# espnet/espnet

Measured on AMD Instinct MI355X. Metric: audio-seconds/sec (RTF^-1), Conformer-ASR, 10 s utterances, higher is better.
Workload: dtype bf16; 1 GPU; BASELINE.json configs[1]: Conformer-small (12x256d, 4 heads), HIP STFT/log-mel + HIP encoder + greedy CTC (G1) + hypotheses collated to the host, 32 x 10 s utterances per GPU per step, V=5000; batch_per_gpu=32, global_batch=32, parallelism=utterance-dp1

## Files before the change

### espnet_amd/csrc/api.hip

```cpp
#include <stdlib.h>

#include <atomic>
#include <mutex>

#include "em_common.h"
#include "switches.h"

namespace {
EmSwitches read_switches() {
  auto on = [](const char* n) { return getenv(n) != nullptr; };
  auto num = [](const char* n, int dflt) { const char* e = getenv(n); return e ? atoi(e) : dflt; };
  EmSwitches s = {};
  s.attn2_stamps = on("EM_ATTN2_STAMPS"); s.block_stamps = on("EM_BLOCK_STAMPS"); s.ffn_stamps = on("EM_FFN_STAMPS");
  s.sub2_stamps = on("EM_SUB2_STAMPS");
  s.block_no_helpers = on("ESPNET_AMD_BLOCK_NO_HELPERS");
  s.sa_split = num("ESPNET_AMD_SA_SPLIT", 0); s.sa_group = num("ESPNET_AMD_SA_GROUP", 0);
  s.no_sa_tree = on("ESPNET_AMD_NO_SA_TREE"); s.sa_tree_min_rows = num("ESPNET_AMD_SA_TREE_MIN_ROWS", 200);
  s.no_attn2_large = on("ESPNET_AMD_NO_ATTN2_LARGE"); s.no_ffn_rows = on("ESPNET_AMD_NO_FFN_ROWS");
  s.no_rows_ctc = on("ESPNET_AMD_NO_ROWS_CTC"); s.frontend_v1 = on("ESPNET_AMD_FRONTEND_V1");
  s.gemm_stages = num("ESPNET_AMD_GEMM_STAGES", 0); s.gemm_bm = num("ESPNET_AMD_GEMM_BM", 0); s.no_mid_gemm = on("ESPNET_AMD_NO_MID_GEMM");
  s.mid_tile = num("ESPNET_AMD_MID_TILE", 0); s.lng_rt = num("ESPNET_AMD_LNG_RT", 0); s.lng_wide = num("ESPNET_AMD_LNG_WIDE", 256);
  s.no_src_lnq = on("ESPNET_AMD_NO_SRC_LNQ"); s.no_tail_fusion = on("ESPNET_AMD_NO_TAIL_FUSION");
  s.stream_no_fused = on("ESPNET_AMD_STREAM_NO_FUSED"); s.stream_mha_v1 = on("ESPNET_AMD_STREAM_MHA_V1");
  s.stream_no_ctx_fold = on("ESPNET_AMD_STREAM_NO_CTX_FOLD"); s.stream_no_ln_gemm = on("ESPNET_AMD_STREAM_NO_LN_GEMM");
  s.stream_fused_min = num("ESPNET_AMD_STREAM_FUSED_MIN", 1); s.no_sub12 = on("ESPNET_AMD_NO_SUB12");
  s.stream_ffn_split = num("ESPNET_AMD_STREAM_FFN_SPLIT", 0); s.stream_split_att = on("ESPNET_AMD_STREAM_SPLIT_ATT");
  s.stream_tf_merge = num("ESPNET_AMD_STREAM_TF_MERGE", -1);
  s.dec_ffn_split = num("ESPNET_AMD_DEC_FFN_SPLIT", 0); s.dec_ffn_rows = num("ESPNET_AMD_DEC_FFN_ROWS", 0); s.no_rows_qkv = on("ESPNET_AMD_NO_ROWS_QKV"); s.ffn_rows_min_fill = num("ESPNET_AMD_FFN_ROWS_MIN_FILL", 0);
  return s;
}
std::atomic<const EmSwitches*> g_sw{nullptr};
std::mutex g_sw_mu;
}

const EmSwitches& em_sw() {
  const EmSwitches* p = g_sw.load(std::memory_order_acquire);
  if (!p) {
    std::lock_guard<std::mutex> lk(g_sw_mu);
    p = g_sw.load(std::memory_order_acquire);
    if (!p) {
      p = new EmSwitches(read_switches());
      g_sw.store(p, std::memory_order_release);
    }
  }
  return *p;
}
extern "C" void em_dev_switches_reload(void) {
  std::lock_guard<std::mutex> lk(g_sw_mu);
  g_sw.store(new EmSwitches(read_switches()), std::memory_order_release);
}

extern "C" int em_version(void) { return 1; }

extern "C" const char* em_error_string(int code) {
  switch (code) {
    case EM_OK: return "ok";
    case EM_ERR_UNSUPPORTED: return "shape/config outside the MI355X fast path";
    case EM_ERR_BAD_ARG: return "bad argument";
    case EM_ERR_TOO_SHORT: return "utterance too short for Conv2dSubsampling (needs >= 7 frames)";
    case EM_ERR_LAUNCH: return "HIP kernel launch failed";
    case EM_ERR_WORKSPACE: return "workspace too small";
    case EM_ERR_IO: return "file I/O failed";
  }
  return "unknown error";
}

template <typename T>
__global__ void cast_f32_kernel(const float* __restrict__ src, size_t n, T* __restrict__ dst) {
  size_t i = (size_t)blockIdx.x * blockDim.x + threadIdx.x;
  const size_t stride = (size_t)gridDim.x * blockDim.x;
  for (; i < n; i += stride) dst[i] = from_f32<T>(src[i]);
}

extern "C" int em_cast_f32(int dtype, const float* src, size_t n, void* dst, void* stream) {
  if (!src || !dst) return EM_ERR_BAD_ARG;
  if (n == 0) return EM_OK;
  int blocks = (int)((n + 255) / 256);
  if (blocks > 4096) blocks = 4096;
  if (dtype == EM_F32)
    hipLaunchKernelGGL(cast_f32_kernel<float>, dim3(blocks), dim3(256), 0, (hipStream_t)stream, src,
                       n, (float*)dst);
  else if (dtype == EM_BF16)
    hipLaunchKernelGGL(cast_f32_kernel<bf16>, dim3(blocks), dim3(256), 0, (hipStream_t)stream, src,
                       n, (bf16*)dst);
  else
    return EM_ERR_BAD_ARG;
  EM_CHECK_LAUNCH();
  return EM_OK;
}
```

### espnet_amd/csrc/frontend.hip

```cpp
#include <stdlib.h>

#include "em_common.h"
#include <type_traits>
#include "switches.h"

__device__ const float2 EM_TW512[384] = {
#include "twiddle512.inc"
};

__device__ __forceinline__ float2 cmul(float2 a, float2 b) {
  return make_float2(a.x * b.x - a.y * b.y, a.x * b.y + a.y * b.x);
}

__device__ __forceinline__ void bfly4(float2 u[4]) {
  float2 a = make_float2(u[0].x + u[2].x, u[0].y + u[2].y);
  float2 b = make_float2(u[0].x - u[2].x, u[0].y - u[2].y);
  float2 c = make_float2(u[1].x + u[3].x, u[1].y + u[3].y);
  float2 d = make_float2(u[1].x - u[3].x, u[1].y - u[3].y);
  u[0] = make_float2(a.x + c.x, a.y + c.y);
  u[2] = make_float2(a.x - c.x, a.y - c.y);
  u[1] = make_float2(b.x + d.y, b.y - d.x);
  u[3] = make_float2(b.x - d.y, b.y + d.x);
}

__device__ __forceinline__ int reflect_idx(int p, int N) {
  if (p < 0) p = -p;
  if (p >= N) p = 2 * (N - 1) - p;
  return p;
}

__global__ __launch_bounds__(256) void frontend_logmel_kernel(
    const float* __restrict__ wav, int N, int hop, const float* __restrict__ window,
    const float* __restrict__ melw, const int* __restrict__ mel_lo, int mel_maxlen, int n_mels,
    const int* __restrict__ flens, const int* __restrict__ wlens, int T_f,
    float* __restrict__ feats) {
  __shared__ float s_re[4][2][256];
  __shared__ float s_im[4][2][256];
  __shared__ float s_pow[4][264];
  const int wave = threadIdx.x >> 6, lane = threadIdx.x & 63;
  const int b = blockIdx.y;
  const int t_raw = blockIdx.x * 4 + wave;
  const int t = t_raw < T_f ? t_raw : T_f - 1;
  const float* x = wav + (size_t)b * N;
  const int Nb = wlens ? (wlens[b] < N ? wlens[b] : N) : N;
  float(*re)[256] = s_re[wave];
  float(*im)[256] = s_im[wave];

  float2 u[4];
  const int start = t * hop - 256;
#pragma unroll
  for (int m = 0; m < 4; ++m) {
    int n = lane + 64 * m;
    int i0 = reflect_idx(start + 2 * n, Nb), i1 = reflect_idx(start + 2 * n + 1, Nb);
    i0 = i0 < 0 ? 0 : (i0 < N ? i0 : N - 1);
    i1 = i1 < 0 ? 0 : (i1 < N ? i1 : N - 1);
    u[m] = make_float2(x[i0] * window[2 * n], x[i1] * window[2 * n + 1]);
  }
  bfly4(u);
#pragma unroll
  for (int q = 0; q < 4; ++q) {
    re[0][4 * lane + q] = u[q].x;
    im[0][4 * lane + q] = u[q].y;
  }
  __syncthreads();
  int cur = 0;
#pragma unroll
  for (int s = 1; s < 4; ++s) {
    const int p = 1 << (2 * s);
    const int k = lane & (p - 1);
    const int j = ((lane - k) << 2) + k;
    const int twstep = 2 * k * (64 / p);
#pragma unroll
    for (int m = 0; m < 4; ++m) {
      float2 v = make_float2(re[cur][lane + 64 * m], im[cur][lane + 64 * m]);
      u[m] = (m == 0) ? v : cmul(v, EM_TW512[m * twstep]);
    }
    bfly4(u);
#pragma unroll
    for (int q = 0; q < 4; ++q) {
      re[cur ^ 1][j + q * p] = u[q].x;
      im[cur ^ 1][j + q * p] = u[q].y;
    }
    cur ^= 1;
    __syncthreads();
  }
  float* pw = s_pow[wave];
#pragma unroll
  for (int m = 0; m < 5; ++m) {
    int k = lane + 64 * m;
    if (m == 4 && lane != 0) break;
    int ka = k & 255, kb = (256 - k) & 255;
    float2 zk = make_float2(re[cur][ka], im[cur][ka]);
    float2 zc = make_float2(re[cur][kb], -im[cur][kb]);
    float2 e = make_float2(0.5f * (zk.x + zc.x), 0.5f * (zk.y + zc.y));
    float2 dlt = make_float2(zk.x - zc.x, zk.y - zc.y);
    float2 o = make_float2(0.5f * dlt.y, -0.5f * dlt.x);
    float2 w = (k < 384) ? EM_TW512[k] : make_float2(0.f, 0.f);
    float2 xo = cmul(w, o);
    float xr = e.x + xo.x, xi = e.y + xo.y;
    pw[k] = xr * xr + xi * xi;
  }
  __syncthreads();
  const bool valid_frame = t < flens[b];
  if (t_raw < T_f) {
    float* out = feats + ((size_t)b * T_f + t) * n_mels;
    auto band = [&](int m, int s0, int s1) {
      float acc = 0.f;
      const int lo = mel_lo[m];
      for (int s = s0; s < s1; ++s) {
        int k = lo + s;
        k = k < 256 ? k : 256;
        acc = fmaf(pw[k], melw[s * n_mels + m], acc);
      }
      return acc;
    };
    const int nfull = n_mels & ~63;
    for (int m = lane; m < nfull; m += 64) {
      const float acc = fmaxf(band(m, 0, mel_maxlen), 1e-10f);
      out[m] = valid_frame ? logf(acc) : 0.f;
    }
    const int rest = n_mels - nfull;
    if (rest > 16) {
      const int m = nfull + lane;
      if (m < n_mels) {
        const float acc = fmaxf(band(m, 0, mel_maxlen), 1e-10f);
        out[m] = valid_frame ? logf(acc) : 0.f;
      }
    } else if (rest > 0) {
      const int q = lane >> 4, mm = nfull + (lane & 15);
      const int m = mm < n_mels ? mm : n_mels - 1;
      const int per = (mel_maxlen + 3) >> 2;
      const int s0 = q * per, s1 = (s0 + per < mel_maxlen) ? s0 + per : mel_maxlen;
      float acc = band(m, s0, s1);
      {
        const Pair2 p16 = wave_xor16_pair(acc);
        acc = p16.a + p16.b;
        const Pair2 p32 = wave_xor32_pair(acc);
        acc = p32.a + p32.b;
      }
      acc = fmaxf(acc, 1e-10f);
      if (q == 0 && mm < n_mels) out[mm] = valid_frame ? logf(acc) : 0.f;
    }
  }
}


__device__ __forceinline__ int fpad(int i) { return i + ((i >> 5) << 2); }
constexpr int FE_TILE = 288;
constexpr int FE_POW = 320;

template <int ML, int FR>
__global__ __launch_bounds__(256) void frontend_logmel_kernel2(
    const float* __restrict__ wav, int N, int hop, const float* __restrict__ window,
    const float* __restrict__ melw, const int* __restrict__ mel_lo, int mel_maxlen, int n_mels,
    const int* __restrict__ flens, const int* __restrict__ wlens, int T_f,
    float* __restrict__ feats) {
  __shared__ __attribute__((aligned(16))) float s_re[4][2][FE_TILE];
  __shared__ __attribute__((aligned(16))) float s_im[4][2][FE_TILE];
  __shared__ float s_pow[4][FE_POW];
  const int wave = threadIdx.x >> 6, lane = threadIdx.x & 63;
  const int b = blockIdx.y;
  const float* x = wav + (size_t)b * N;
  const int Nb = wlens ? (wlens[b] < N ? wlens[b] : N) : N;
  float(*re)[FE_TILE] = s_re[wave];
  float(*im)[FE_TILE] = s_im[wave];
  float* pw = s_pow[wave];
  const int flen = flens[b];

  float2 win[4];
#pragma unroll
  for (int m = 0; m < 4; ++m) win[m] = *(const float2*)(window + 2 * (lane + 64 * m));
  float2 tw[3][3];
  int jst[3];
#pragma unroll
  for (int s = 1; s < 4; ++s) {
    const int p = 1 << (2 * s);
    const int k = lane & (p - 1);
    jst[s - 1] = fpad(((lane - k) << 2) + k);
    const int twstep = 2 * k * (64 / p);
#pragma unroll
    for (int m = 1; m < 4; ++m) tw[s - 1][m - 1] = EM_TW512[m * twstep];
  }
  const int rd0 = fpad(lane);
  const int kb0 = fpad(256 - lane);
  const int st0 = fpad(4 * lane);
  float2 twu[4];
#pragma unroll
  for (int m = 0; m < 4; ++m) twu[m] = (lane + 64 * m < 384) ? EM_TW512[lane + 64 * m] : make_float2(0.f, 0.f);
  const int nfull = n_mels > 64 ? 64 : 0;
  const int mA = lane < n_mels ? lane : n_mels - 1;
  const int loA = mel_lo[mA];
  float wA[ML];
#pragma unroll
  for (int s = 0; s < ML; ++s) wA[s] = (s < mel_maxlen && loA + s <= 256) ? melw[s * n_mels + mA] : 0.f;
  const int rest = n_mels - nfull;
  (void)rest;
  const int qB = lane >> 4, mmB = nfull + (lane & 15);
  const int mB = mmB < n_mels ? mmB : n_mels - 1;
  const int per = (mel_maxlen + 3) >> 2;
  const int s0B = qB * per, s1B = (s0B + per < mel_maxlen) ? s0B + per : mel_maxlen;
  const int loB = mel_lo[mB] + s0B;
  constexpr int MLB = (ML + 3) / 4;
  float wB[MLB];
#pragma unroll
  for (int s = 0; s < MLB; ++s) wB[s] = (nfull && s0B + s < s1B && loB + s <= 256) ? melw[(s0B + s) * n_mels + mB] : 0.f;
  for (int i = 257 + lane; i < FE_POW; i += 64) pw[i] = 0.f;
  const float* const pwA = pw + loA;
  const float* const pwB = pw + (loB < FE_POW - MLB ? loB : FE_POW - MLB);
  for (int fi = 0; fi < FR; ++fi) {
    const int t = (blockIdx.x * FR + fi) * 4 + wave;
    if (t >= T_f) break;
    float2 u[4];
    const int start = t * hop - 256;
    if (start >= 0 && start + 512 <= Nb && !(((size_t)b * N + start) & 1)) {
#pragma unroll
      for (int m = 0; m < 4; ++m) {
        const float2 v = *(const float2*)(x + start + 2 * (lane + 64 * m));
        u[m] = make_float2(v.x * win[m].x, v.y * win[m].y);
      }
    } else {
#pragma unroll
      for (int m = 0; m < 4; ++m) {
        const int n = lane + 64 * m;
        int i0 = reflect_idx(start + 2 * n, Nb), i1 = reflect_idx(start + 2 * n + 1, Nb);
        i0 = i0 < 0 ? 0 : (i0 < N ? i0 : N - 1);
        i1 = i1 < 0 ? 0 : (i1 < N ? i1 : N - 1);
        u[m] = make_float2(x[i0] * win[m].x, x[i1] * win[m].y);
      }
    }
    bfly4(u);
    *(float4*)(re[0] + st0) = make_float4(u[0].x, u[1].x, u[2].x, u[3].x);
    *(float4*)(im[0] + st0) = make_float4(u[0].y, u[1].y, u[2].y, u[3].y);
    __builtin_amdgcn_wave_barrier();
    int cur = 0;
#pragma unroll
    for (int s = 1; s < 4; ++s) {
      const int p = 1 << (2 * s);
#pragma unroll
      for (int m = 0; m < 4; ++m) {
        const float2 v = make_float2(re[cur][rd0 + 72 * m], im[cur][rd0 + 72 * m]);
        u[m] = (m == 0) ? v : cmul(v, tw[s - 1][m - 1]);
      }
      bfly4(u);
#pragma unroll
      for (int q = 0; q < 4; ++q) {
        const int off = p == 4 ? 4 * q : (p == 16 ? 16 * q + 4 * (q >> 1) : 72 * q);
        re[cur ^ 1][jst[s - 1] + off] = u[q].x;
        im[cur ^ 1][jst[s - 1] + off] = u[q].y;
      }
      cur ^= 1;
      __builtin_amdgcn_wave_barrier();
    }
#pragma unroll
    for (int m = 0; m < 5; ++m) {
      const int k = lane + 64 * m;
      if (m == 4 && lane != 0) break;
      const int pa = m < 4 ? rd0 + 72 * m : 0;
      const int pb = m == 0 ? (lane == 0 ? 0 : kb0) : (m < 4 ? kb0 - 72 * m : 0);
      const float2 zk = make_float2(re[cur][pa], im[cur][pa]);
      const float2 zc = make_float2(re[cur][pb], -im[cur][pb]);
      const float2 e = make_float2(0.5f * (zk.x + zc.x), 0.5f * (zk.y + zc.y));
      const float2 dlt = make_float2(zk.x - zc.x, zk.y - zc.y);
      const float2 o = make_float2(0.5f * dlt.y, -0.5f * dlt.x);
      const float2 w = m < 4 ? twu[m] : EM_TW512[256];
      const float2 xo = cmul(w, o);
      const float xr = e.x + xo.x, xi = e.y + xo.y;
      pw[k] = xr * xr + xi * xi;
    }
    __builtin_amdgcn_wave_barrier();
    const bool valid_frame = t < flen;
    float* out = feats + ((size_t)b * T_f + t) * n_mels;
    {
      float acc = 0.f;
#pragma unroll
      for (int s = 0; s < ML; ++s) acc = fmaf(pwA[s], wA[s], acc);
      acc = fmaxf(acc, 1e-10f);
      if (lane < n_mels) out[lane] = valid_frame ? logf(acc) : 0.f;
    }
    if (nfull) {
      float acc = 0.f;
#pragma unroll
      for (int s = 0; s < MLB; ++s) acc = fmaf(pwB[s], wB[s], acc);
      {
        const Pair2 p16 = wave_xor16_pair(acc);
        acc = p16.a + p16.b;
        const Pair2 p32 = wave_xor32_pair(acc);
        acc = p32.a + p32.b;
      }
      acc = fmaxf(acc, 1e-10f);
      if (qB == 0 && mmB < n_mels) out[mmB] = valid_frame ? logf(acc) : 0.f;
    }
    __builtin_amdgcn_wave_barrier();
  }
}

extern "C" int em_frontend_logmel_f32(const float* wav, int32_t B, int32_t N, int32_t hop,
                                      const float* window, const float* mel_packed,
                                      const int32_t* mel_lo, int32_t mel_maxlen, int32_t n_mels,
                                      const int32_t* flens, const int32_t* wlens, int32_t T_f,
                                      float* feats, void* stream) {
  if (B <= 0 || T_f <= 0) return EM_ERR_BAD_ARG;
  if (N <= 256 || hop <= 0 || T_f != 1 + N / hop) return EM_ERR_BAD_ARG;
  if (mel_maxlen < 1 || mel_maxlen > 257 || n_mels < 1) return EM_ERR_BAD_ARG;
  const bool v1 = em_sw().frontend_v1;
  if (!v1 && mel_maxlen <= 32 && n_mels <= 80) {
    auto launch = [&](auto ml_c, auto fr_c) {
      constexpr int ML = decltype(ml_c)::value, FR = decltype(fr_c)::value;
      dim3 grid(em_cdiv(T_f, 4 * FR), B);
      hipLaunchKernelGGL((frontend_logmel_kernel2<ML, FR>), grid, dim3(256), 0, (hipStream_t)stream, wav, N, hop, window,
                         mel_packed, mel_lo, mel_maxlen, n_mels, flens, wlens, T_f, feats);
    };
    const bool few = (long)em_cdiv(T_f, 32) * B < 256;
    using I2 = std::integral_constant<int, 2>;
    using I8 = std::integral_constant<int, 8>;
    using I20 = std::integral_constant<int, 20>;
    using I32 = std::integral_constant<int, 32>;
    if (mel_maxlen <= 20) {
      if (few) launch(I20{}, I2{});
      else launch(I20{}, I8{});
    } else {
      if (few) launch(I32{}, I2{});
      else launch(I32{}, I8{});
    }
    EM_CHECK_LAUNCH();
    return EM_OK;
  }
  dim3 grid(em_cdiv(T_f, 4), B);
  hipLaunchKernelGGL(frontend_logmel_kernel, grid, dim3(256), 0, (hipStream_t)stream, wav, N, hop,
                     window, mel_packed, mel_lo, mel_maxlen, n_mels, flens, wlens, T_f, feats);
  EM_CHECK_LAUNCH();
  return EM_OK;
}

__global__ __launch_bounds__(256) void utt_mvn_partial_kernel(const float* __restrict__ feats,
                                                              const int* __restrict__ flens,
                                                              int T_f, int n_mels,
                                                              float* __restrict__ partial) {
  __shared__ float s_acc[256];
  const int b = blockIdx.y, part = blockIdx.x;
  const int len = flens[b] < T_f ? flens[b] : T_f;
  const int chunk = (len + 7) / 8;
  const int t0 = part * chunk;
  const int t1 = (t0 + chunk) < len ? (t0 + chunk) : len;
  if (n_mels > 256) {
    for (int m = threadIdx.x; m < n_mels; m += blockDim.x) {
      float acc = 0.f;
      for (int t = t0; t < t1; ++t) acc += feats[((size_t)b * T_f + t) * n_mels + m];
      partial[((size_t)b * 8 + part) * n_mels + m] = acc;
    }
    return;
  }
  if (n_mels % 4 == 0 && n_mels <= 256) {
    const int C4 = n_mels >> 2;
    const int FL4 = 256 / C4;
    const int fl = threadIdx.x / C4, c = threadIdx.x - fl * C4;
    float4 acc = make_float4(0.f, 0.f, 0.f, 0.f);
    if (fl < FL4) {
      const float4* base = (const float4*)(feats + (size_t)b * T_f * n_mels) + c;
      for (int t = t0 + fl; t < t1; t += 4 * FL4) {
        float4 v[4];
#pragma unroll
        for (int u = 0; u < 4; ++u) {
          const int tt = t + u * FL4;
          v[u] = base[(size_t)(tt < t1 ? tt : t1 - 1) * C4];
        }
#pragma unroll
        for (int u = 0; u < 4; ++u)
          if (t + u * FL4 < t1) {
            acc.x += v[u].x; acc.y += v[u].y; acc.z += v[u].z; acc.w += v[u].w;
          }
      }
    }
    __shared__ float4 s_acc4[256];
    s_acc4[threadIdx.x] = acc;
    __syncthreads();
    if (threadIdx.x < C4) {
      float4 tot = make_float4(0.f, 0.f, 0.f, 0.f);
      for (int q = 0; q < FL4; ++q) {
        const float4 a = s_acc4[q * C4 + threadIdx.x];
        tot.x += a.x; tot.y += a.y; tot.z += a.z; tot.w += a.w;
      }
      *(float4*)(partial + ((size_t)b * 8 + part) * n_mels + 4 * threadIdx.x) = tot;
    }
    return;
  }
  const int FL = 256 / n_mels;
  const int fl = threadIdx.x / n_mels, m = threadIdx.x - fl * n_mels;
  float acc = 0.f;
  if (fl < FL)
    for (int t = t0 + fl; t < t1; t += FL) acc += feats[((size_t)b * T_f + t) * n_mels + m];
  s_acc[threadIdx.x] = acc;
  __syncthreads();
  if (threadIdx.x < n_mels) {
    float tot = 0.f;
    for (int q = 0; q < FL; ++q) tot += s_acc[q * n_mels + threadIdx.x];
    partial[((size_t)b * 8 + part) * n_mels + threadIdx.x] = tot;
  }
}

extern "C" int em_utt_mvn_partial_f32(const float* feats, const int32_t* flens, int32_t B,
                                      int32_t T_f, int32_t n_mels, float* partial, void* stream) {
  if (B <= 0 || T_f <= 0 || n_mels <= 0) return EM_ERR_BAD_ARG;
  hipLaunchKernelGGL(utt_mvn_partial_kernel, dim3(8, B), dim3(256), 0, (hipStream_t)stream, feats,
                     flens, T_f, n_mels, partial);
  EM_CHECK_LAUNCH();
  return EM_OK;
}

template <typename T>
__global__ __launch_bounds__(256) void conv2d_sub1_kernel(
    const float* __restrict__ feats, const float* __restrict__ partial,
    const int* __restrict__ flens, int T_f, int n_mels, const float* __restrict__ w1,
    const float* __restrict__ b1, int d, int T1, int F1, T* __restrict__ out) {
  __shared__ float s_in[3][128];
  const int t1 = blockIdx.x, b = blockIdx.y;
  for (int i = threadIdx.x; i < 3 * n_mels; i += blockDim.x) {
    int r = i / n_mels, f = i - r * n_mels;
    float mean = 0.f;
    if (partial) {
      const float* pp = partial + (size_t)b * 8 * n_mels + f;
      float s = 0.f;
#pragma unroll
      for (int q = 0; q < 8; ++q) s += pp[q * n_mels];
      mean = s / (float)flens[b];
    }
    s_in[r][f] = feats[((size_t)b * T_f + 2 * t1 + r) * n_mels + f] - mean;
  }
  __syncthreads();
  for (int c = threadIdx.x; c < d; c += blockDim.x) {
    float w[9];
#pragma unroll
    for (int i = 0; i < 9; ++i) w[i] = w1[c * 9 + i];
    const float bias = b1[c];
    T* o = out + ((size_t)(b * T1 + t1) * F1) * d + c;
    for (int f1 = 0; f1 < F1; ++f1) {
      float acc = bias;
#pragma unroll
      for (int i = 0; i < 3; ++i)
#pragma unroll
        for (int j = 0; j < 3; ++j) acc = fmaf(w[i * 3 + j], s_in[i][2 * f1 + j], acc);
      o[(size_t)f1 * d] = from_f32<T>(fmaxf(acc, 0.f));
    }
  }
}

extern "C" int em_conv2d_sub1(int dtype, const float* feats, const float* partial,
                              const int32_t* flens, int32_t B, int32_t T_f, int32_t n_mels,
                              const float* w1, const float* b1, int32_t d, void* out,
                              void* stream) {
  if (B <= 0 || n_mels < 3 || n_mels > 128 || d <= 0) return EM_ERR_BAD_ARG;
  if (T_f < 7) return EM_ERR_TOO_SHORT;
  const int T1 = (T_f - 3) / 2 + 1, F1 = (n_mels - 3) / 2 + 1;
  dim3 grid(T1, B);
  if (dtype == EM_F32)
    hipLaunchKernelGGL(conv2d_sub1_kernel<float>, grid, dim3(256), 0, (hipStream_t)stream, feats,
                       partial, flens, T_f, n_mels, w1, b1, d, T1, F1, (float*)out);
  else if (dtype == EM_BF16)
    hipLaunchKernelGGL(conv2d_sub1_kernel<bf16>, grid, dim3(256), 0, (hipStream_t)stream, feats,
                       partial, flens, T_f, n_mels, w1, b1, d, T1, F1, (bf16*)out);
  else
    return EM_ERR_BAD_ARG;
  EM_CHECK_LAUNCH();
  return EM_OK;
}

__global__ __launch_bounds__(256) void global_mvn_kernel(float* __restrict__ x,
                                                         const int* __restrict__ flens,
                                                         const float* __restrict__ mean,
                                                         const float* __restrict__ stdv, int T_f,
                                                         int n_mels) {
  const int b = blockIdx.y;
  const size_t n = (size_t)T_f * n_mels;
  float* xb = x + (size_t)b * n;
  const int len = flens ? flens[b] : T_f;
  for (size_t i = (size_t)blockIdx.x * 256 + threadIdx.x; i < n; i += (size_t)gridDim.x * 256) {
    const int t = (int)(i / n_mels), c = (int)(i - (size_t)t * n_mels);
    float v = xb[i];
    if (mean) v -= mean[c];
    if (t >= len) v = 0.f;
    if (stdv) v /= stdv[c];
    xb[i] = v;
  }
}

extern "C" int em_global_mvn_f32(float* feats, const int32_t* flens, const float* mean,
                                 const float* stdv, int32_t B, int32_t T_f, int32_t n_mels,
                                 void* stream) {
  if (!feats || B <= 0 || T_f <= 0 || n_mels <= 0) return EM_ERR_BAD_ARG;
  int gx = (int)(((size_t)T_f * n_mels + 255) / 256);
  gx = gx > 256 ? 256 : gx;
  hipLaunchKernelGGL(global_mvn_kernel, dim3(gx, B), dim3(256), 0, (hipStream_t)stream, feats, flens,
                     mean, stdv, T_f, n_mels);
  EM_CHECK_LAUNCH();
  return EM_OK;
}

__global__ __launch_bounds__(256) void utt_mvn_apply_kernel(float* __restrict__ x,
                                                            const float* __restrict__ partial,
                                                            const int* __restrict__ flens, int T_f,
                                                            int n_mels) {
  const int b = blockIdx.y;
  const size_t n = (size_t)T_f * n_mels;
  float* xb = x + (size_t)b * n;
  const int len = flens[b];
  for (size_t i = (size_t)blockIdx.x * 256 + threadIdx.x; i < n; i += (size_t)gridDim.x * 256) {
    const int t = (int)(i / n_mels), c = (int)(i - (size_t)t * n_mels);
    const float* pp = partial + (size_t)b * 8 * n_mels + c;
    float sm = 0.f;
#pragma unroll
    for (int q = 0; q < 8; ++q) sm += pp[q * n_mels];
    xb[i] = (t < len ? xb[i] : 0.f) - sm / (float)len;
  }
}

extern "C" int em_utt_mvn_apply_f32(float* feats, const float* partial, const int32_t* flens,
                                    int32_t B, int32_t T_f, int32_t n_mels, void* stream) {
  if (!feats || !partial || !flens || B <= 0 || T_f <= 0 || n_mels <= 0) return EM_ERR_BAD_ARG;
  int gx = (int)(((size_t)T_f * n_mels + 255) / 256);
  gx = gx > 256 ? 256 : gx;
  hipLaunchKernelGGL(utt_mvn_apply_kernel, dim3(gx, B), dim3(256), 0, (hipStream_t)stream, feats,
                     partial, flens, T_f, n_mels);
  EM_CHECK_LAUNCH();
  return EM_OK;
}
```

### espnet_amd/csrc/switches.h

```cpp
#pragma once

struct EmSwitches {
  bool attn2_stamps, block_stamps, ffn_stamps, sub2_stamps;
  bool block_no_helpers;
  int sa_split, sa_group;
  bool no_sa_tree;
  int sa_tree_min_rows;
  bool no_rows_qkv;
  bool no_attn2_large, no_ffn_rows, no_rows_ctc;
  bool frontend_v1;
  int gemm_stages, gemm_bm;
  bool no_mid_gemm;
  int mid_tile, lng_rt, lng_wide;
  bool no_src_lnq, no_tail_fusion;
  bool stream_no_fused, stream_mha_v1, stream_no_ctx_fold, stream_no_ln_gemm;
  int stream_fused_min;
  bool stream_split_att;
  int stream_ffn_split;
  int stream_tf_merge;
  bool no_sub12;
  int ffn_rows_min_fill;
  int dec_ffn_rows;
  int dec_ffn_split;
};

const EmSwitches& em_sw();
```

Before: 362,100 audio-s/s.

## Add packed-math radix-4 FFT log-mel kernel with frame prefetch; deepen CMVN unroll

```diff
diff --git a/espnet_amd/csrc/api.hip b/espnet_amd/csrc/api.hip
--- a/espnet_amd/csrc/api.hip
+++ b/espnet_amd/csrc/api.hip
@@ -18,6 +18,7 @@
   s.no_sa_tree = on("ESPNET_AMD_NO_SA_TREE"); s.sa_tree_min_rows = num("ESPNET_AMD_SA_TREE_MIN_ROWS", 200);
   s.no_attn2_large = on("ESPNET_AMD_NO_ATTN2_LARGE"); s.no_ffn_rows = on("ESPNET_AMD_NO_FFN_ROWS");
   s.no_rows_ctc = on("ESPNET_AMD_NO_ROWS_CTC"); s.frontend_v1 = on("ESPNET_AMD_FRONTEND_V1");
+  s.frontend_v2 = on("ESPNET_AMD_FRONTEND_V2");
   s.gemm_stages = num("ESPNET_AMD_GEMM_STAGES", 0); s.gemm_bm = num("ESPNET_AMD_GEMM_BM", 0); s.no_mid_gemm = on("ESPNET_AMD_NO_MID_GEMM");
   s.mid_tile = num("ESPNET_AMD_MID_TILE", 0); s.lng_rt = num("ESPNET_AMD_LNG_RT", 0); s.lng_wide = num("ESPNET_AMD_LNG_WIDE", 256);
   s.no_src_lnq = on("ESPNET_AMD_NO_SRC_LNQ"); s.no_tail_fusion = on("ESPNET_AMD_NO_TAIL_FUSION");
diff --git a/espnet_amd/csrc/frontend.hip b/espnet_amd/csrc/frontend.hip
--- a/espnet_amd/csrc/frontend.hip
+++ b/espnet_amd/csrc/frontend.hip
@@ -294,6 +294,205 @@
   }
 }
 
+typedef float f2v __attribute__((ext_vector_type(2)));
+typedef float f4v __attribute__((ext_vector_type(4)));
+__device__ __forceinline__ int fpad3(int i) { return i + ((i >> 4) << 1); }
+constexpr int FE3_TILE = 288;
+
+__device__ __forceinline__ f2v cmul_tw(f2v v, f2v txx, f2v tny) {
+#pragma clang fp contract(off)
+  const f2v p = v.yx * tny;
+  return __builtin_elementwise_fma(v, txx, p);
+}
+__device__ __forceinline__ f2v add_pm(f2v x, f2v y) { return __builtin_elementwise_fma(y, (f2v){1.f, -1.f}, x); }
+__device__ __forceinline__ f2v add_mp(f2v x, f2v y) { return __builtin_elementwise_fma(y, (f2v){-1.f, 1.f}, x); }
+__device__ __forceinline__ void bfly4_tail(f2v u[4], f2v a, f2v b, f2v c, f2v d) {
+#pragma clang fp contract(off)
+  u[0] = a + c;
+  u[2] = a - c;
+  u[1] = add_pm(b, d.yx);
+  u[3] = add_mp(b, d.yx);
+}
+
+template <int ML, int FR>
+__global__ __launch_bounds__(256) __attribute__((amdgpu_waves_per_eu(ML <= 20 ? 4 : 3))) void frontend_logmel_kernel3(
+    const float* __restrict__ wav, int N, int hop, const float* __restrict__ window,
+    const float* __restrict__ melw, const int* __restrict__ mel_lo, int mel_maxlen, int n_mels,
+    const int* __restrict__ flens, const int* __restrict__ wlens, int T_f,
+    float* __restrict__ feats) {
+#pragma clang fp contract(off)
+  __shared__ __attribute__((aligned(16))) f2v s_z[4][2][FE3_TILE];
+  __shared__ float s_pow[4][FE_POW];
+  const int wave = threadIdx.x >> 6, lane = threadIdx.x & 63;
+  const int b = blockIdx.y;
+  const float* x = wav + (size_t)b * N;
+  const int Nb = wlens ? (wlens[b] < N ? wlens[b] : N) : N;
+  f2v(*z)[FE3_TILE] = s_z[wave];
+  float* pw = s_pow[wave];
+  const int flen = flens[b];
+
+  f2v win[4];
+#pragma unroll
+  for (int m = 0; m < 4; ++m) win[m] = *(const f2v*)(window + 2 * (lane + 64 * m));
+  f2v txa[3], txb[3], tny[3][3], wx3, wny[4];
+#pragma unroll
+  for (int m = 0; m < 4; ++m) {
+    const float2 w = (lane + 64 * m < 384) ? EM_TW512[lane + 64 * m] : make_float2(0.f, 0.f);
+    wny[m] = (f2v){-w.y, w.y};
+    if (m < 3) txb[m].y = w.x;
+    else wx3 = (f2v){w.x, w.x};
+  }
+  int jst[3];
+#pragma unroll
+  for (int s = 1; s < 4; ++s) {
+    const int p = 1 << (2 * s);
+    const int k = lane & (p - 1);
+    jst[s - 1] = fpad3(((lane - k) << 2) + k);
+    const int twstep = 2 * k * (64 / p);
+#pragma unroll
+    for (int m = 1; m < 4; ++m) {
+      const float2 t = EM_TW512[m * twstep];
+      tny[s - 1][m - 1] = (f2v){-t.y, t.y};
+      if (m == 1) txa[s - 1].x = t.x;
+      else if (m == 2) txa[s - 1].y = t.x;
+      else txb[s - 1].x = t.x;
+    }
+  }
+  const int rd0 = fpad3(lane);
+  const int kb0 = fpad3(256 - lane);
+  const int st0 = fpad3(4 * lane);
+  const int nfull = n_mels > 64 ? 64 : 0;
+  const int mA = lane < n_mels ? lane : n_mels - 1;
+  const int loA = mel_lo[mA];
+  float wA[ML];
+#pragma unroll
+  for (int s = 0; s < ML; ++s) wA[s] = (s < mel_maxlen && loA + s <= 256) ? melw[s * n_mels + mA] : 0.f;
+  const int qB = lane >> 4, mmB = nfull + (lane & 15);
+  const int mB = mmB < n_mels ? mmB : n_mels - 1;
+  const int per = (mel_maxlen + 3) >> 2;
+  const int s0B = qB * per, s1B = (s0B + per < mel_maxlen) ? s0B + per : mel_maxlen;
+  const int loB = mel_lo[mB] + s0B;
+  constexpr int MLB = (ML + 3) / 4;
+  float wB[MLB];
+#pragma unroll
+  for (int s = 0; s < MLB; ++s) wB[s] = (nfull && s0B + s < s1B && loB + s <= 256) ? melw[(s0B + s) * n_mels + mB] : 0.f;
+  for (int i = 257 + lane; i < FE_POW; i += 64) pw[i] = 0.f;
+  const float* const pwA = pw + loA;
+  const float* const pwB = pw + (loB < FE_POW - MLB ? loB : FE_POW - MLB);
+  auto load_frame = [&](int t, f2v(&xo)[4]) {
+    const int start = t * hop - 256;
+    if (start >= 0 && start + 512 <= Nb && !(((size_t)b * N + start) & 1)) {
+      int n0 = start + 2 * lane;
+      asm volatile("" : "+v"(n0));
+      const f2v* xa = (const f2v*)(x + n0);
+#pragma unroll
+      for (int m = 0; m < 4; ++m) xo[m] = xa[64 * m];
+    } else {
+#pragma unroll
+      for (int m = 0; m < 4; ++m) {
+        const int n = lane + 64 * m;
+        int i0 = reflect_idx(start + 2 * n, Nb), i1 = reflect_idx(start + 2 * n + 1, Nb);
+        i0 = i0 < 0 ? 0 : (i0 < N ? i0 : N - 1);
+        i1 = i1 < 0 ? 0 : (i1 < N ? i1 : N - 1);
+        xo[m] = (f2v){x[i0], x[i1]};
+      }
+    }
+  };
+  f2v xn[4] = {};
+  if ((int)(blockIdx.x * FR * 4 + wave) < T_f) load_frame(blockIdx.x * FR * 4 + wave, xn);
+#pragma unroll 1
+  for (int fi = 0; fi < FR; ++fi) {
+    const int t = (blockIdx.x * FR + fi) * 4 + wave;
+    if (t >= T_f) break;
+    asm volatile("" : "+v"(txa[0]), "+v"(txa[1]), "+v"(txa[2]), "+v"(txb[0]), "+v"(txb[1]), "+v"(txb[2]));
+    f2v xv[4], u[4];
+#pragma unroll
+    for (int m = 0; m < 4; ++m) xv[m] = xn[m];
+    if (fi + 1 < FR && t + 4 < T_f) load_frame(t + 4, xn);
+    {
+      const f2v p2 = xv[2] * win[2], p3 = xv[3] * win[3];
+      f2v a = __builtin_elementwise_fma(xv[0], win[0], p2);
+      a.y = xv[0].y * win[0].y + p2.y;
+      const f2v bb = __builtin_elementwise_fma(xv[0], win[0], -p2);
+      const f2v c = __builtin_elementwise_fma(xv[1], win[1], p3);
+      const f2v d = __builtin_elementwise_fma(xv[1], win[1], -p3);
+      bfly4_tail(u, a, bb, c, d);
+    }
+    *(f4v*)(z[0] + st0) = (f4v){u[0].x, u[0].y, u[1].x, u[1].y};
+    *(f4v*)(z[0] + st0 + 2) = (f4v){u[2].x, u[2].y, u[3].x, u[3].y};
+    __builtin_amdgcn_wave_barrier();
+    int cur = 0;
+#pragma unroll
+    for (int s = 1; s < 4; ++s) {
+      const int p = 1 << (2 * s);
+#pragma unroll
+      for (int m = 0; m < 4; ++m) {
+        const f2v v = z[cur][rd0 + 72 * m];
+        u[m] = m == 0 ? v : cmul_tw(v, m == 1 ? txa[s - 1].xx : (m == 2 ? txa[s - 1].yy : txb[s - 1].xx), tny[s - 1][m > 0 ? m - 1 : 0]);
+      }
+      bfly4_tail(u, u[0] + u[2], u[0] - u[2], u[1] + u[3], u[1] - u[3]);
+#pragma unroll
+      for (int q = 0; q < 4; ++q) {
+        const int off = p == 4 ? 4 * q : (p == 16 ? 18 * q : 72 * q);
+        z[cur ^ 1][jst[s - 1] + off] = u[q];
+      }
+      cur ^= 1;
+      __builtin_amdgcn_wave_barrier();
+    }
+    f2v zk[4], zb[4];
+#pragma unroll
+    for (int m = 0; m < 4; ++m) {
+      zk[m] = z[cur][rd0 + 72 * m];
+      zb[m] = z[cur][m == 0 ? (lane == 0 ? 0 : kb0) : kb0 - 72 * m];
+    }
+    asm volatile("" : "+v"(zk[2]), "+v"(zb[2]), "+v"(zk[3]), "+v"(zb[3]));
+#pragma unroll
+    for (int m = 0; m < 5; ++m) {
+      const int k = lane + 64 * m;
+      if (m == 4 && lane != 0) break;
+      const f2v sm = add_pm(zk[m & 3], zb[m & 3]);
+      const f2v dl = add_mp(zk[m & 3], zb[m & 3]);
+      const f2v o = dl.yx * (f2v){0.5f, -0.5f};
+      const float2 w256 = EM_TW512[256];
+      const f2v xo = m < 3 ? cmul_tw(o, txb[m].yy, wny[m])
+                           : (m == 3 ? cmul_tw(o, wx3, wny[3]) : cmul_tw(o, (f2v){w256.x, w256.x}, (f2v){-w256.y, w256.y}));
+      const f2v X = __builtin_elementwise_fma((f2v){0.5f, 0.5f}, sm, xo);
+      pw[k] = m < 4 ? __builtin_fmaf(X.x, X.x, X.y * X.y) : X.x * X.x + X.y * X.y;
+    }
+    __builtin_amdgcn_wave_barrier();
+    const bool valid_frame = t < flen;
+    float* out = feats + ((size_t)b * T_f + t) * n_mels;
+    float pA[ML], pB[MLB];
+#pragma unroll
+    for (int s = 0; s < ML; ++s) pA[s] = pwA[s];
+#pragma unroll
+    for (int s = 0; s < MLB; ++s) pB[s] = pwB[s];
+    if constexpr (ML == 20)
+      asm volatile("" : "+v"(pA[0]), "+v"(pA[1]), "+v"(pA[2]), "+v"(pA[3]), "+v"(pA[4]), "+v"(pA[5]), "+v"(pA[6]), "+v"(pA[7]), "+v"(pA[8]), "+v"(pA[9]), "+v"(pA[10]), "+v"(pA[11]), "+v"(pA[12]), "+v"(pA[13]), "+v"(pA[14]), "+v"(pA[15]), "+v"(pA[16]), "+v"(pA[17]), "+v"(pA[18]), "+v"(pA[19]), "+v"(pB[0]), "+v"(pB[1]), "+v"(pB[2]), "+v"(pB[3]), "+v"(pB[4]));
+    {
+      float acc = 0.f;
+#pragma unroll
+      for (int s = 0; s < ML; ++s) acc = fmaf(pA[s], wA[s], acc);
+      acc = fmaxf(acc, 1e-10f);
+      if (lane < n_mels) out[lane] = valid_frame ? logf(acc) : 0.f;
+    }
+    if (nfull) {
+      float acc = 0.f;
+#pragma unroll
+      for (int s = 0; s < MLB; ++s) acc = fmaf(pB[s], wB[s], acc);
+      {
+        const Pair2 p16 = wave_xor16_pair(acc);
+        acc = p16.a + p16.b;
+        const Pair2 p32 = wave_xor32_pair(acc);
+        acc = p32.a + p32.b;
+      }
+      acc = fmaxf(acc, 1e-10f);
+      if (qB == 0 && mmB < n_mels) out[mmB] = valid_frame ? logf(acc) : 0.f;
+    }
+    __builtin_amdgcn_wave_barrier();
+  }
+}
+
 extern "C" int em_frontend_logmel_f32(const float* wav, int32_t B, int32_t N, int32_t hop,
                                       const float* window, const float* mel_packed,
                                       const int32_t* mel_lo, int32_t mel_maxlen, int32_t n_mels,
@@ -303,12 +502,17 @@
   if (N <= 256 || hop <= 0 || T_f != 1 + N / hop) return EM_ERR_BAD_ARG;
   if (mel_maxlen < 1 || mel_maxlen > 257 || n_mels < 1) return EM_ERR_BAD_ARG;
   const bool v1 = em_sw().frontend_v1;
+  const bool v2 = em_sw().frontend_v2;
   if (!v1 && mel_maxlen <= 32 && n_mels <= 80) {
     auto launch = [&](auto ml_c, auto fr_c) {
       constexpr int ML = decltype(ml_c)::value, FR = decltype(fr_c)::value;
       dim3 grid(em_cdiv(T_f, 4 * FR), B);
-      hipLaunchKernelGGL((frontend_logmel_kernel2<ML, FR>), grid, dim3(256), 0, (hipStream_t)stream, wav, N, hop, window,
-                         mel_packed, mel_lo, mel_maxlen, n_mels, flens, wlens, T_f, feats);
+      if (v2)
+        hipLaunchKernelGGL((frontend_logmel_kernel2<ML, FR>), grid, dim3(256), 0, (hipStream_t)stream, wav, N, hop, window,
+                           mel_packed, mel_lo, mel_maxlen, n_mels, flens, wlens, T_f, feats);
+      else
+        hipLaunchKernelGGL((frontend_logmel_kernel3<ML, FR>), grid, dim3(256), 0, (hipStream_t)stream, wav, N, hop, window,
+                           mel_packed, mel_lo, mel_maxlen, n_mels, flens, wlens, T_f, feats);
     };
     const bool few = (long)em_cdiv(T_f, 32) * B < 256;
     using I2 = std::integral_constant<int, 2>;
@@ -351,21 +555,22 @@
     return;
   }
   if (n_mels % 4 == 0 && n_mels <= 256) {
+    constexpr int NF = 12;
     const int C4 = n_mels >> 2;
     const int FL4 = 256 / C4;
     const int fl = threadIdx.x / C4, c = threadIdx.x - fl * C4;
     float4 acc = make_float4(0.f, 0.f, 0.f, 0.f);
     if (fl < FL4) {
       const float4* base = (const float4*)(feats + (size_t)b * T_f * n_mels) + c;
-      for (int t = t0 + fl; t < t1; t += 4 * FL4) {
-        float4 v[4];
-#pragma unroll
-        for (int u = 0; u < 4; ++u) {
+      for (int t = t0 + fl; t < t1; t += NF * FL4) {
+        float4 v[NF];
+#pragma unroll
+        for (int u = 0; u < NF; ++u) {
           const int tt = t + u * FL4;
           v[u] = base[(size_t)(tt < t1 ? tt : t1 - 1) * C4];
         }
 #pragma unroll
-        for (int u = 0; u < 4; ++u)
+        for (int u = 0; u < NF; ++u)
           if (t + u * FL4 < t1) {
             acc.x += v[u].x; acc.y += v[u].y; acc.z += v[u].z; acc.w += v[u].w;
           }
diff --git a/espnet_amd/csrc/switches.h b/espnet_amd/csrc/switches.h
--- a/espnet_amd/csrc/switches.h
+++ b/espnet_amd/csrc/switches.h
@@ -8,7 +8,7 @@
   int sa_tree_min_rows;
   bool no_rows_qkv;
   bool no_attn2_large, no_ffn_rows, no_rows_ctc;
-  bool frontend_v1;
+  bool frontend_v1, frontend_v2;
   int gemm_stages, gemm_bm;
   bool no_mid_gemm;
   int mid_tile, lng_rt, lng_wide;
```

New measurement: 361,600 audio-s/s. About the same (-0.1%).
